# AdaptiveCity/deepdish

Measured on AMD Instinct MI355X. Metric: end-to-end frames/sec (detect+encode+track) at 640x480, higher is better.
Workload: dtype i8 (reference: uint8); encoder f16; 1 GPU; SSD-MobileNet-v1 uint8-quantised (300x300) + MARS-64x32x3 + deep_sort on synthetic 640x480 BGR frames, ~20 synthetic detections/frame (BASELINE.json configs[1]); streams_per_gpu=3072, worker_threads_per_gpu=2, parallelism=independent streams, 3072 per GPU in 2 worker groups, weights=seeded synthetic (seed 1234)

## Files before the change

### deepdish_amd/csrc/mars_pair.hip

```cpp
#include "mars_tail.h"

namespace {

typedef _Float16 h8 __attribute__((ext_vector_type(8)));
typedef float f4 __attribute__((ext_vector_type(4)));
typedef unsigned u4 __attribute__((ext_vector_type(4)));

__device__ __forceinline__ float elu(float v) {
    float e = __builtin_amdgcn_exp2f(v * 1.44269504088896340736f);
    e = __builtin_amdgcn_fmed3f(e, 0.f, 1.f);
    return __builtin_amdgcn_fmed3f(v, e - 1.f, 3.0e38f);
}

__device__ __forceinline__ void lds_fill16(const _Float16 *g, char *lds_wave_base) {
#if defined(__HIP_DEVICE_COMPILE__)
    __builtin_amdgcn_global_load_lds(g, lds_wave_base, 16, 0, 0);
#endif
}

__device__ __forceinline__ int frag_row(int a, int fr) { return (fr >> 2) * 8 + (a & 1) * 4 + (fr & 3); }

constexpr int PZ_B = 3072;
constexpr int PT64_B = 18 * 1024;
constexpr int PT32_B = 33 * 1024;
constexpr int PPLAIN_B = 16 * 1024;
constexpr int PRAW_B = 8 * 1024;
constexpr int pair_off_in(bool) { return PZ_B; }
constexpr int pair_off_h(bool first) { return PZ_B + 2 * (first ? PT32_B : PT64_B); }
constexpr int pair_off_res(bool first) { return pair_off_h(first) + 2 * PT64_B; }
constexpr int pair_off_raw(bool first) { return pair_off_res(first) + (first ? 2 : 3) * PPLAIN_B; }
constexpr int pair_off_const(bool first) { return pair_off_raw(first) + (first ? 2 * PRAW_B : 0); }
constexpr int pair_lds_bytes(bool first) { return pair_off_const(first) + 5 * 64 * 4; }

template <bool FIRST>
__global__ __launch_bounds__(512, 2) void mars_pair64_k(const MarsPairP P) {
    constexpr int OFF_IN = pair_off_in(FIRST), OFF_H = pair_off_h(FIRST), OFF_RES = pair_off_res(FIRST), OFF_RAW = pair_off_raw(FIRST),
                  OFF_C = pair_off_const(FIRST);
    constexpr int TIN_B = FIRST ? PT32_B : PT64_B, NRES = FIRST ? 2 : 3;
    extern __shared__ __attribute__((aligned(16))) char smem[];
    const int tid = threadIdx.x, lane = tid & 63;
    const int wave = __builtin_amdgcn_readfirstlane(tid >> 6);
    const int stage = wave >> 2, half = wave & 1, q = (wave >> 1) & 1;
    const int fr = lane & 15, fq = lane >> 4, j = fr >> 3, x = fr & 7;

    for (int i = tid * 16; i < OFF_C; i += 512 * 16) *reinterpret_cast<u4 *>(smem + i) = u4{0u, 0u, 0u, 0u};
    float *cst = reinterpret_cast<float *>(smem + OFF_C);
    if (tid < 64) {
        cst[tid] = P.bias_a[tid];
        cst[64 + tid] = P.bias_b[tid];
        cst[128 + tid] = P.aff2[tid];
        cst[192 + tid] = P.aff2[P.cout_pad + tid];
        cst[256 + tid] = (FIRST && P.bias_p) ? P.bias_p[tid] : 0.f;
    }
    __syncthreads();

    h8 wf[9][2][2];
    h8 wp[2];
    const bool a32 = FIRST && stage == 0;
    {
        const _Float16 *w = stage == 0 ? P.wa : P.wb;
        const int kpad = stage == 0 ? P.kpad_a : P.kpad_b;
#pragma unroll
        for (int t = 0; t < 9; ++t)
#pragma unroll
            for (int ks = 0; ks < 2; ++ks)
#pragma unroll
                for (int a = 0; a < 2; ++a) {
                    const size_t row = (size_t)(half * 32 + frag_row(a, fr)) * kpad;
                    wf[t][ks][a] = a32 ? *reinterpret_cast<const h8 *>(w + row + t * 32 + fq * 8)
                                       : *reinterpret_cast<const h8 *>(w + row + t * 64 + ks * 32 + fq * 8);
                }
#pragma unroll
        for (int a = 0; a < 2; ++a)
// ... 16 lines not shown
    size_t stp[5];
    int n_dma;
    if constexpr (FIRST) {
        const int par = lane >> 5, pl = (lane >> 3) & 3, col = 2 * (lane & 7) + par;
#pragma unroll
        for (int h = 0; h < 4; ++h) {
            const int r = wave + 8 * h < 31 ? wave + 8 * h : 30;
            src[h] = col < 15 ? P.in + ((size_t)n0 * 31 + r) * 15 * P.cs_in + (size_t)col * P.cs_in + P.coff_in + pl * 8 : P.zero;
            stp[h] = col < 15 ? (size_t)nstep * 31 * 15 * P.cs_in : 0;
        }
        const int jr = lane >> 5, xx = lane & 7;
        src[4] = P.in2 + ((size_t)n0 * 31 + 2 * (2 * wave + jr)) * 15 * P.cs_in2 + (size_t)(2 * xx) * P.cs_in2 + P.coff_in2 + pl * 8;
        stp[4] = (size_t)nstep * 31 * 15 * P.cs_in2;
        n_dma = 5;
    } else {
        const int pl = lane >> 3, xx = lane & 7;
#pragma unroll
        for (int h = 0; h < 2; ++h) {
            src[h] = P.in + (((size_t)n0 * 16 + wave + 8 * h) * 8 + xx) * P.cs_in + P.coff_in + pl * 8;
            stp[h] = (size_t)nstep * 128 * P.cs_in;
            src[2 + h] = P.res + (((size_t)n0 * 16 + wave + 8 * h) * 8 + xx) * P.cs_res + P.coff_res + pl * 8;
            stp[2 + h] = (size_t)nstep * 128 * P.cs_res;
        }
        src[4] = P.zero; stp[4] = 0;
        n_dma = 4;
    }
    (void)n_dma;
    int dq = 0;
    auto issue = [&]() {
        char *T = smem + OFF_IN + (dq & 1) * TIN_B;
        if constexpr (FIRST) {
#pragma unroll
            for (int h = 0; h < 4; ++h) lds_fill16(src[h], T + ((wave + 8 * h < 31 ? wave + 8 * h : 30) + 1) * 1024);
            lds_fill16(src[4], smem + OFF_RAW + (dq & 1) * PRAW_B + wave * 1024);
        } else {
#pragma unroll
            for (int h = 0; h < 2; ++h) lds_fill16(src[h], T + (wave + 8 * h + 1) * 1024);
            const int rs = dq % 3;
#pragma unroll
            for (int h = 0; h < 2; ++h) lds_fill16(src[2 + h], smem + OFF_RES + rs * PPLAIN_B + (wave + 8 * h) * 1024);
        }
        ++dq;
        const bool more = dq < Kc;
#pragma unroll
        for (int h = 0; h < 5; ++h) src[h] += more ? stp[h] : 0;
    };

    const int co = half * 32 + fq * 8;
    const unsigned lo64 = (unsigned)((j * 64 + fq * 8 + x) * 16);
    const unsigned lo32 = (unsigned)((2 * j * 64 + fq * 8 + x) * 16);
    const f4 ba0 = *reinterpret_cast<const f4 *>(cst + (stage ? 64 : 0) + co), ba1 = *reinterpret_cast<const f4 *>(cst + (stage ? 64 : 0) + co + 4);

    issue();
    for (int c = 0; c <= Kc; ++c) {
#if defined(__HIP_DEVICE_COMPILE__)
        if (stage == 0 || c < 2) asm volatile("s_waitcnt vmcnt(0) lgkmcnt(0)" ::: "memory");
        else asm volatile("s_waitcnt vmcnt(8) lgkmcnt(0)" ::: "memory");
        __builtin_amdgcn_s_barrier();
        asm volatile("" ::: "memory");
#endif
        issue();
        const int cc = stage == 0 ? c : c - 1;
        if (cc < 0 || cc >= Kc) continue;
        const size_t n = (size_t)(n0 + cc * nstep);
#pragma unroll 1
        for (int f = 0; f < 4; ++f) {
            const int F = 4 * q + f;
            f4 acc[2] = {f4{0.f, 0.f, 0.f, 0.f}, f4{0.f, 0.f, 0.f, 0.f}};
            h8 X[4];
            if (a32) {
                const unsigned tb = (unsigned)(OFF_IN + (cc & 1) * PT32_B + 4 * F * 1024) + lo32;
                const unsigned bL = x == 0 ? ((tb + 512u - 16u) & 255u) : tb + 512u - 16u, bC = tb, bR = tb + 512u;
                const unsigned pb = (unsigned)(OFF_RAW + (cc & 1) * PRAW_B) + (unsigned)(((2 * F + j) * 32 + fq * 8 + x) * 16);
                f4 accp[2] = {f4{0.f, 0.f, 0.f, 0.f}, f4{0.f, 0.f, 0.f, 0.f}};
#if defined(__HIP_DEVICE_COMPILE__)
#define DD_RD(u_) do { if constexpr ((u_) < 9) { constexpr int dy_ = (u_) / 3, dx_ = (u_) - dy_ * 3;                                               \
                           asm volatile("ds_read_b128 %0, %1 offset:%2" : "=&v"(X[(u_) & 3]) : "v"(dx_ == 0 ? bL : dx_ == 1 ? bC : bR), "n"(dy_ * 1024) : "memory"); } \
                       else asm volatile("ds_read_b128 %0, %1" : "=&v"(X[(u_) & 3]) : "v"(pb) : "memory"); } while (0)
#define DD_UNIT(u_) do { if constexpr ((u_) + 3 < 10) DD_RD(((u_) + 3) % 10);                                                                      \
                         asm volatile("s_waitcnt lgkmcnt(%1)" : "+v"(X[(u_) & 3]) : "n"((u_) + 3 < 10 ? 3 : 9 - (u_)));                           \
                         if constexpr ((u_) < 9) { _Pragma("unroll") for (int a = 0; a < 2; ++a) acc[a] = __builtin_amdgcn_mfma_f32_16x16x32_f16(wf[(u_) % 9][0][a], X[(u_) & 3], acc[a], 0, 0, 0); } \
                         else { _Pragma("unroll") for (int a = 0; a < 2; ++a) accp[a] = __builtin_amdgcn_mfma_f32_16x16x32_f16(wp[a], X[(u_) & 3], accp[a], 0, 0, 0); } } while (0)
                DD_RD(0); DD_RD(1); DD_RD(2);
                DD_UNIT(0); DD_UNIT(1); DD_UNIT(2); DD_UNIT(3); DD_UNIT(4); DD_UNIT(5); DD_UNIT(6); DD_UNIT(7); DD_UNIT(8); DD_UNIT(9);
#undef DD_UNIT
#undef DD_RD
#endif
                const f4 c0 = *reinterpret_cast<const f4 *>(cst + 256 + co), c1 = *reinterpret_cast<const f4 *>(cst + 256 + co + 4);
                h8 sk;
#pragma unroll
                for (int i = 0; i < 4; ++i) { sk[i] = (_Float16)(accp[0][i] + c0[i]); sk[4 + i] = (_Float16)(accp[1][i] + c1[i]); }
                *reinterpret_cast<h8 *>(smem + OFF_RES + (cc & 1) * PPLAIN_B + ((2 * F + j) * 64 + (half * 4 + fq) * 8 + x) * 16) = sk;
            } else {
                const unsigned tb = (unsigned)((stage == 0 ? OFF_IN + (cc & 1) * PT64_B : OFF_H + (cc & 1) * PT64_B) + 2 * F * 1024) + lo64;
                const unsigned bL = x == 0 ? ((tb - 16u) & 255u) : tb - 16u, bC = tb, bR = x == 7 ? ((tb + 16u) & 255u) : tb + 16u;
#if defined(__HIP_DEVICE_COMPILE__)
#define DD_RD(u_) do { constexpr int t_ = (u_) >> 1, ks_ = (u_) & 1, dy_ = t_ / 3, dx_ = t_ - dy_ * 3;                                             \
                       asm volatile("ds_read_b128 %0, %1 offset:%2" : "=&v"(X[(u_) & 3]) : "v"(dx_ == 0 ? bL : dx_ == 1 ? bC : bR), "n"(dy_ * 1024 + ks_ * 512) : "memory"); } while (0)
#define DD_UNIT(u_) do { if constexpr ((u_) + 3 < 18) DD_RD(((u_) + 3) % 18);                                                                      \
                         asm volatile("s_waitcnt lgkmcnt(%1)" : "+v"(X[(u_) & 3]) : "n"((u_) + 3 < 18 ? 3 : 17 - (u_)));                          \
                         _Pragma("unroll") for (int a = 0; a < 2; ++a) acc[a] = __builtin_amdgcn_mfma_f32_16x16x32_f16(wf[(u_) >> 1][(u_) & 1][a], X[(u_) & 3], acc[a], 0, 0, 0); } while (0)
                DD_RD(0); DD_RD(1); DD_RD(2);
                DD_UNIT(0); DD_UNIT(1); DD_UNIT(2); DD_UNIT(3); DD_UNIT(4); DD_UNIT(5); DD_UNIT(6); DD_UNIT(7); DD_UNIT(8);
                DD_UNIT(9); DD_UNIT(10); DD_UNIT(11); DD_UNIT(12); DD_UNIT(13); DD_UNIT(14); DD_UNIT(15); DD_UNIT(16); DD_UNIT(17);
#undef DD_UNIT
#undef DD_RD
#endif
            }
            float v[8];
#pragma unroll
            for (int i = 0; i < 4; ++i) { v[i] = acc[0][i] + ba0[i]; v[4 + i] = acc[1][i] + ba1[i]; }
            if (stage == 0) {
                h8 o;
#pragma unroll
                for (int i = 0; i < 8; ++i) o[i] = (_Float16)elu(v[i]);
                *reinterpret_cast<h8 *>(smem + OFF_H + (cc & 1) * PT64_B + ((2 * F + j + 1) * 64 + (half * 4 + fq) * 8 + x) * 16) = o;
            } else {
                const int rs = FIRST ? (cc & 1) : cc % 3;
                const h8 rv = *reinterpret_cast<const h8 *>(smem + OFF_RES + rs * PPLAIN_B + ((2 * F + j) * 64 + (half * 4 + fq) * 8 + x) * 16);
#pragma unroll
                for (int i = 0; i < 8; ++i) v[i] += (float)rv[i];
                const size_t m = (n * 16 + 2 * F + j) * 8 + x;
                h8 o;
#pragma unroll
                for (int i = 0; i < 8; ++i) o[i] = (_Float16)v[i];
                *reinterpret_cast<h8 *>(P.out + m * P.cs_out + P.coff_out + co) = o;
                const f4 s0 = *reinterpret_cast<const f4 *>(cst + 128 + co), s1 = *reinterpret_cast<const f4 *>(cst + 128 + co + 4);
                const f4 t0 = *reinterpret_cast<const f4 *>(cst + 192 + co), t1 = *reinterpret_cast<const f4 *>(cst + 192 + co + 4);
                h8 o2;
#pragma unroll
                for (int i = 0; i < 4; ++i) { o2[i] = (_Float16)elu(s0[i] * v[i] + t0[i]); o2[4 + i] = (_Float16)elu(s1[i] * v[4 + i] + t1[i]); }
                *reinterpret_cast<h8 *>(P.out2 + m * P.cs_out2 + P.coff_out2 + co) = o2;
            }
        }
    }
#if defined(__HIP_DEVICE_COMPILE__)
    asm volatile("s_waitcnt vmcnt(0)" ::: "memory");
#endif
}

template <bool FIRST>
int launch_pair(hipStream_t s, int device, const MarsPairP &P) {
    constexpr int lds = pair_lds_bytes(FIRST);
    static_assert(lds <= 160 * 1024, "LDS budget");
    static DevOnce once;
    const int rc = once.run(device, [&]() -> int {
        DD_HIP(hipFuncSetAttribute(reinterpret_cast<const void *>(&mars_pair64_k<FIRST>), hipFuncAttributeMaxDynamicSharedMemorySize, lds));
        return DD_OK;
    });
    if (rc != DD_OK) return rc;
    const int n_cu = dd_cu_count(device);
    const int grid = P.n_img < n_cu ? P.n_img : n_cu;
    hipLaunchKernelGGL((mars_pair64_k<FIRST>), dim3(grid), dim3(512), lds, s, P);
    DD_LAUNCH_CHECK();
    return DD_OK;
}

}

int mars_pair64_launch(hipStream_t s, int device, const MarsPairP &P, bool first) {
    DD_REQUIRE(P.n_img > 0 && P.in && P.wa && P.wb && P.bias_a && P.bias_b && P.out && P.out2 && P.aff2 && P.zero && (first ? (P.in2 && P.wp) : P.res != nullptr), DD_E_ARG,
               "mars_pair64: bad argument");
    return first ? launch_pair<true>(s, device, P) : launch_pair<false>(s, device, P);
}
```

### deepdish_amd/csrc/mars_tail.hip

```cpp
#include "mars_tail.h"
#include <vector>

namespace {

typedef _Float16 h8 __attribute__((ext_vector_type(8)));
typedef float f4 __attribute__((ext_vector_type(4)));
typedef unsigned u4 __attribute__((ext_vector_type(4)));

enum { ACT_NONE = 0, ACT_ELU = 2 };

__device__ __forceinline__ float elu(float v) {
    float e = __builtin_amdgcn_exp2f(v * 1.44269504088896340736f);
    e = __builtin_amdgcn_fmed3f(e, 0.f, 1.f);
    return __builtin_amdgcn_fmed3f(v, e - 1.f, 3.0e38f);
}

__device__ __forceinline__ void lds_fill16(const _Float16 *g, char *lds_wave_base) {
#if defined(__HIP_DEVICE_COMPILE__)
    __builtin_amdgcn_global_load_lds(g, lds_wave_base, 16, 0, 0);
#endif
}

__device__ __forceinline__ int frag_row(int a, int fr) { return (fr >> 2) * 8 + (a & 1) * 4 + (fr & 3); }

#ifdef DD_MARS_STAMPS
__device__ unsigned long long dd_mars_stamps[256 * 8 * 8];
#define DD_STAMP(k) do { const unsigned long long t_ = __builtin_amdgcn_s_memtime(); st_acc[k] += t_ - st_last; st_last = t_; } while (0)
#else
#define DD_STAMP(k) do { } while (0)
#endif

constexpr int WS_LEAD = 2, WS_NB = WS_LEAD + 2, WS_NBR = WS_LEAD + 3;
constexpr int ws_tile_bytes(int mode) { return mode == MARS_WS_S2_PROJ ? 17 * 68 * 16 : 10 * 72 * 16; }
constexpr int ws_zero_bytes(int mode) { return mode == MARS_WS_S2_PROJ ? 0 : 7680; }
constexpr int WS_RES_BYTES = 8 * 72 * 16, WS_PRJ_BYTES = 4096;
constexpr int ws_xw_bytes(int mode) { return mode == MARS_WS_S2_PROJ ? 4096 : 2048; }
constexpr int ws_off_tiles(int mode) { return ws_zero_bytes(mode); }
constexpr int ws_off_aux(int mode) { return ws_off_tiles(mode) + WS_NB * ws_tile_bytes(mode); }
constexpr int ws_off_xchg(int mode) {
    return ws_off_aux(mode) + (mode == MARS_WS_S1_RES ? WS_NBR * WS_RES_BYTES : mode == MARS_WS_S2_PROJ ? WS_NB * WS_PRJ_BYTES : 0);
}
constexpr int ws_off_const(int mode) { return ws_off_xchg(mode) + 2 * 8 * ws_xw_bytes(mode); }
constexpr int ws_lds_bytes(int mode) { return ws_off_const(mode) + 3 * 128 * 4; }

template <int MODE, int ACT, bool OUT2>
__global__ __launch_bounds__(512, 2) void mars_ws128_k(const MarsWsP P) {
    constexpr bool S2 = MODE == MARS_WS_S2_PROJ, RES = MODE == MARS_WS_S1_RES;
    constexpr int LEAD = WS_LEAD, NB = WS_NB, NBR = WS_NBR;
    constexpr int TILE_B = ws_tile_bytes(MODE), XW_B = ws_xw_bytes(MODE);
    constexpr int OFF_T = ws_off_tiles(MODE), OFF_A = ws_off_aux(MODE), OFF_X = ws_off_xchg(MODE), OFF_C = ws_off_const(MODE);
    constexpr int KS = S2 ? 1 : 2, CIN = S2 ? 64 : 128;
    [[maybe_unused]] constexpr int N_DMA = S2 ? 3 : RES ? 2 : 1;
    [[maybe_unused]] constexpr int N_ST = S2 ? 2 : (RES && OUT2) ? 2 : 1;
    extern __shared__ __attribute__((aligned(16))) char smem[];
    const int tid = threadIdx.x, lane = tid & 63;
    const int wave = __builtin_amdgcn_readfirstlane(tid >> 6);
    const int cg = wave & 3, kh = wave >> 2;
    const int fr = lane & 15, fq = lane >> 4, yy = fr >> 2, x = fr & 3;

    for (int i = tid * 16; i < OFF_A; i += 512 * 16) *reinterpret_cast<u4 *>(smem + i) = u4{0u, 0u, 0u, 0u};
    float *cst = reinterpret_cast<float *>(smem + OFF_C);
    if (tid < 128) {
        cst[tid] = P.bias[tid];
        if constexpr (S2) cst[128 + tid] = P.bias2 ? P.bias2[tid] : 0.f;
        if constexpr (RES && OUT2) { cst[128 + tid] = P.aff2[tid]; cst[256 + tid] = P.aff2[P.cout_pad + tid]; }
    }
    __syncthreads();

    h8 wf[9][KS][2];
#pragma unroll
    for (int t = 0; t < 9; ++t)
#pragma unroll
        for (int ks = 0; ks < KS; ++ks)
#pragma unroll
            for (int a = 0; a < 2; ++a)
                wf[t][ks][a] = *reinterpret_cast<const h8 *>(P.w + (size_t)(cg * 32 + frag_row(a, fr)) * P.kpad + t * CIN + kh * (CIN / 2) + ks * 32 + fq * 8);
    h8 wp[2];
    if constexpr (S2) {
#pragma unroll
        for (int a = 0; a < 2; ++a) wp[a] = *reinterpret_cast<const h8 *>(P.w2 + (size_t)(cg * 32 + frag_row(a, fr)) * P.kpad2 + kh * 32 + fq * 8);
    }

#if defined(__HIP_DEVICE_COMPILE__)
#pragma unroll
    for (int t = 0; t < 9; ++t)
#pragma unroll
        for (int ks = 0; ks < KS; ++ks)
#pragma unroll
            for (int a = 0; a < 2; ++a) asm volatile("" ::"v"(wf[t][ks][a]));
    if constexpr (S2) asm volatile("" ::"v"(wp[0]), "v"(wp[1]));
#endif

    const int n0 = blockIdx.x, nstep = gridDim.x;
    const int Kc = (P.n_img - n0 + nstep - 1) / nstep;

    int dq = 0, dq_slot = 0, dq_rslot = 0;
    const _Float16 *src_a, *src_b, *src_c;
    size_t step_a, step_b, step_c;
    if constexpr (!S2) {
        src_a = P.in + (size_t)n0 * 32 * P.cs_in + ((wave * 4 + (lane & 3)) * P.cs_in + P.coff_in + (lane >> 2) * 8);
        src_b = RES ? P.res + (size_t)n0 * 32 * P.cs_res + ((wave * 4 + (lane & 3)) * P.cs_res + P.coff_res + (lane >> 2) * 8) : P.zero;
        src_c = P.zero;
        step_a = (size_t)nstep * 32 * P.cs_in; step_b = (size_t)nstep * 32 * P.cs_res; step_c = 0;
    } else {
        const int par = lane >> 5, pl = (lane >> 2) & 7, col = 2 * (lane & 3) + par;
        src_a = P.in + (size_t)n0 * 128 * P.cs_in + ((wave * 8 + col) * P.cs_in + P.coff_in + pl * 8);
        src_b = src_a + (size_t)64 * P.cs_in;
        const int ch = (wave & 3) * 64 + lane;
        src_c = P.in2 + (size_t)n0 * 128 * P.cs_in2 + ((2 * ((ch >> 2) & 7) * 8 + 2 * (ch & 3)) * P.cs_in2 + P.coff_in2 + (ch >> 5) * 8);
        step_a = step_b = (size_t)nstep * 128 * P.cs_in; step_c = (size_t)nstep * 128 * P.cs_in2;
    }
    auto issue = [&]() {
        char *T = smem + OFF_T + dq_slot * TILE_B;
        if constexpr (!S2) {
            lds_fill16(src_a, T + (wave + 1) * 72 * 16);
            if constexpr (RES) lds_fill16(src_b, smem + OFF_A + dq_rslot * WS_RES_BYTES + wave * 72 * 16);
        } else {
            lds_fill16(src_a, T + wave * 68 * 16);
            lds_fill16(src_b, T + (wave + 8) * 68 * 16);
            lds_fill16(src_c, smem + OFF_A + dq_slot * WS_PRJ_BYTES + (wave & 3) * 1024);
        }
        ++dq;
        const bool more = dq < Kc;
        src_a += more ? step_a : 0;
        if constexpr (RES || S2) src_b += more ? step_b : 0;
        if constexpr (S2) src_c += more ? step_c : 0;
        dq_slot = dq_slot + 1 == NB ? 0 : dq_slot + 1;
        dq_rslot = dq_rslot + 1 == NBR ? 0 : dq_rslot + 1;
    };

    const unsigned lo = S2 ? (unsigned)((2 * yy * 68 + (kh * 4 + fq) * 4 + x) * 16) : (unsigned)((yy * 72 + (kh * 8 + fq) * 4 + x) * 16);
    const unsigned lo_prj = (unsigned)(((kh * 4 + fq) * 32 + yy * 4 + x) * 16);
    const unsigned lo_res = (unsigned)(((4 * kh + yy) * 72 + (cg * 4 + fq) * 4 + x) * 16);
    const int co = cg * 32 + fq * 8;
    const f4 b0 = *reinterpret_cast<const f4 *>(cst + co), b1 = *reinterpret_cast<const f4 *>(cst + co + 4);

    f4 keep[S2 ? 4 : 2];
    int slot = 0, rslot_prev = 0, rslot = 0;

    auto epilogue = [&](int cprev) {
        const char *Xp = smem + OFF_X + ((cprev & 1) * 8 + (wave ^ 4)) * XW_B + lane * 16;
        const size_t n = (size_t)(n0 + cprev * nstep);
        const size_t m = (n * 8 + 4 * kh + yy) * 4 + x;
        float v[8];
        {
            const f4 o0 = *reinterpret_cast<const f4 *>(Xp), o1 = *reinterpret_cast<const f4 *>(Xp + 1024);
#pragma unroll
            for (int i = 0; i < 4; ++i) { v[i] = keep[0][i] + o0[i] + b0[i]; v[4 + i] = keep[1][i] + o1[i] + b1[i]; }
        }
        if constexpr (ACT == ACT_ELU) {
#pragma unroll
            for (int i = 0; i < 8; ++i) v[i] = elu(v[i]);
        }
        if constexpr (RES) {
            const h8 rv = *reinterpret_cast<const h8 *>(smem + OFF_A + rslot_prev * WS_RES_BYTES + lo_res);
#pragma unroll
            for (int i = 0; i < 8; ++i) v[i] += (float)rv[i];
        }
        h8 o;
#pragma unroll
        for (int i = 0; i < 8; ++i) o[i] = (_Float16)v[i];
        *reinterpret_cast<h8 *>(P.out + m * P.cs_out + P.coff_out + co) = o;
        if constexpr (RES && OUT2) {
            const f4 s0 = *reinterpret_cast<const f4 *>(cst + 128 + co), s1 = *reinterpret_cast<const f4 *>(cst + 128 + co + 4);
            const f4 t0 = *reinterpret_cast<const f4 *>(cst + 256 + co), t1 = *reinterpret_cast<const f4 *>(cst + 256 + co + 4);
            h8 o2;
#pragma unroll
            for (int i = 0; i < 4; ++i) { o2[i] = (_Float16)elu(s0[i] * v[i] + t0[i]); o2[4 + i] = (_Float16)elu(s1[i] * v[4 + i] + t1[i]); }
            *reinterpret_cast<h8 *>(P.out2 + m * P.cs_out2 + P.coff_out2 + co) = o2;
        }
        if constexpr (S2) {
            const f4 o0 = *reinterpret_cast<const f4 *>(Xp + 2048), o1 = *reinterpret_cast<const f4 *>(Xp + 3072);
            const f4 c0 = *reinterpret_cast<const f4 *>(cst + 128 + co), c1 = *reinterpret_cast<const f4 *>(cst + 128 + co + 4);
            h8 o2;
#pragma unroll
            for (int i = 0; i < 4; ++i) { o2[i] = (_Float16)(keep[2][i] + o0[i] + c0[i]); o2[4 + i] = (_Float16)(keep[3][i] + o1[i] + c1[i]); }
            *reinterpret_cast<h8 *>(P.out2 + m * P.cs_out2 + P.coff_out2 + co) = o2;
        }
    };

#ifdef DD_MARS_STAMPS
    unsigned long long st_acc[8] = {0, 0, 0, 0, 0, 0, 0, 0}, st_last = __builtin_amdgcn_s_memtime();
    const unsigned long long st_begin = st_last;
#endif
    static_assert(LEAD == 2, "the counted waits below are written for two crops of look-ahead");
    for (int ci = 0; ci < LEAD; ++ci) issue();
    DD_STAMP(0);
    for (int c = 0; c <= Kc; ++c) {
#if defined(__HIP_DEVICE_COMPILE__)
        if (kh == 0 || c == 0) {
            if (c <= 1) asm volatile("s_waitcnt vmcnt(%0) lgkmcnt(0)" ::"i"(N_DMA) : "memory");
            else if (c == 2) asm volatile("s_waitcnt vmcnt(%0) lgkmcnt(0)" ::"i"(N_DMA + N_ST) : "memory");
            else asm volatile("s_waitcnt vmcnt(%0) lgkmcnt(0)" ::"i"(N_DMA + 2 * N_ST) : "memory");
        } else asm volatile("s_waitcnt lgkmcnt(0)" ::: "memory");
        DD_STAMP(2);
        __builtin_amdgcn_s_barrier();
        asm volatile("" ::: "memory");
#endif
        DD_STAMP(3);
        auto compute = [&](f4 (&kp)[S2 ? 4 : 2]) {
            const unsigned tb = (unsigned)(OFF_T + slot * TILE_B) + lo;
            f4 acc[2][2] = {{f4{0.f, 0.f, 0.f, 0.f}, f4{0.f, 0.f, 0.f, 0.f}}, {f4{0.f, 0.f, 0.f, 0.f}, f4{0.f, 0.f, 0.f, 0.f}}};
            if constexpr (!S2) {
                const unsigned bs[3] = {x == 0 ? ((tb - 16u) & 255u) : tb - 16u, tb, x == 3 ? ((tb + 16u) & 255u) : tb + 16u};
                h8 X[4][2];
#if defined(__HIP_DEVICE_COMPILE__)
#define DD_RD(u_) do { constexpr int t_ = (u_) >> 1, p_ = (u_) & 1, dy_ = t_ / 3, dx_ = t_ - dy_ * 3;                                      \
                       asm volatile("ds_read_b128 %0, %2 offset:%3\n\tds_read_b128 %1, %2 offset:%4"                                       \
                                    : "=&v"(X[(u_) & 3][0]), "=&v"(X[(u_) & 3][1]) : "v"(bs[dx_]), "n"(((4 * p_ + dy_) * 72) * 16), "n"(((4 * p_ + dy_) * 72 + 16) * 16) : "memory"); } while (0)
#define DD_UNIT(u_) do { if constexpr ((u_) + 3 < 18) DD_RD(((u_) + 3) % 18);                                                            \
                         asm volatile("s_waitcnt lgkmcnt(%2)" : "+v"(X[(u_) & 3][0]), "+v"(X[(u_) & 3][1]) : "n"((u_) + 3 < 18 ? 6 : 2 * (17 - (u_))));          \
                         _Pragma("unroll") for (int ks = 0; ks < 2; ++ks) _Pragma("unroll") for (int a = 0; a < 2; ++a)                  \
                             acc[(u_) & 1][a] = __builtin_amdgcn_mfma_f32_16x16x32_f16(wf[(u_) >> 1][ks][a], X[(u_) & 3][ks], acc[(u_) & 1][a], 0, 0, 0); } while (0)
                DD_RD(0); DD_RD(1); DD_RD(2);
                DD_UNIT(0); DD_UNIT(1); DD_UNIT(2); DD_UNIT(3); DD_UNIT(4); DD_UNIT(5); DD_UNIT(6); DD_UNIT(7); DD_UNIT(8);
                DD_UNIT(9); DD_UNIT(10); DD_UNIT(11); DD_UNIT(12); DD_UNIT(13); DD_UNIT(14); DD_UNIT(15); DD_UNIT(16); DD_UNIT(17);
#undef DD_UNIT
#undef DD_RD
#endif
            } else {
                f4 accp[2][2] = {{f4{0.f, 0.f, 0.f, 0.f}, f4{0.f, 0.f, 0.f, 0.f}}, {f4{0.f, 0.f, 0.f, 0.f}, f4{0.f, 0.f, 0.f, 0.f}}};
                h8 X[4];
                const unsigned pb = (unsigned)(OFF_A + slot * WS_PRJ_BYTES) + lo_prj;
                const h8 hz = {(_Float16)0.f, (_Float16)0.f, (_Float16)0.f, (_Float16)0.f, (_Float16)0.f, (_Float16)0.f, (_Float16)0.f, (_Float16)0.f};
#if defined(__HIP_DEVICE_COMPILE__)
#define DD_RD(u_) do { if constexpr ((u_) < 18) { constexpr int t_ = (u_) >> 1, p_ = (u_) & 1, dy_ = t_ / 3, dx_ = t_ - dy_ * 3;                    \
                           asm volatile("ds_read_b128 %0, %1 offset:%2" : "=&v"(X[(u_) & 3]) : "v"(tb), "n"(((8 * p_ + dy_) * 68 + (dx_ == 1 ? 32 : 0) + (dx_ == 2 ? 1 : 0)) * 16) : "memory"); } \
                       else asm volatile("ds_read_b128 %0, %1 offset:%2" : "=&v"(X[(u_) & 3]) : "v"(pb), "n"(((u_) - 18) * 256) : "memory"); } while (0)
#define DD_UNIT(u_) do { if constexpr ((u_) + 3 < 20) DD_RD(((u_) + 3) % 20);                                                            \
                         asm volatile("s_waitcnt lgkmcnt(%1)" : "+v"(X[(u_) & 3]) : "n"((u_) + 3 < 20 ? 3 : 19 - (u_)));               \
                         if constexpr ((u_) < 18) { const h8 xv_ = (((u_) >> 1) % 3 == 2 && x == 3) ? hz : X[(u_) & 3];                    \
                             _Pragma("unroll") for (int a = 0; a < 2; ++a) acc[(u_) & 1][a] = __builtin_amdgcn_mfma_f32_16x16x32_f16(wf[(u_) >> 1][0][a], xv_, acc[(u_) & 1][a], 0, 0, 0); } \
                         else { _Pragma("unroll") for (int a = 0; a < 2; ++a) accp[(u_) - 18][a] = __builtin_amdgcn_mfma_f32_16x16x32_f16(wp[a], X[(u_) & 3], accp[(u_) - 18][a], 0, 0, 0); } } while (0)
                DD_RD(0); DD_RD(1); DD_RD(2);
                DD_UNIT(0); DD_UNIT(1); DD_UNIT(2); DD_UNIT(3); DD_UNIT(4); DD_UNIT(5); DD_UNIT(6); DD_UNIT(7); DD_UNIT(8); DD_UNIT(9);
                DD_UNIT(10); DD_UNIT(11); DD_UNIT(12); DD_UNIT(13); DD_UNIT(14); DD_UNIT(15); DD_UNIT(16); DD_UNIT(17); DD_UNIT(18); DD_UNIT(19);
#undef DD_UNIT
#undef DD_RD
#endif
                char *Xm = smem + OFF_X + ((c & 1) * 8 + wave) * XW_B + lane * 16;
                *reinterpret_cast<f4 *>(Xm + 2048) = kh ? accp[0][0] : accp[1][0];
                *reinterpret_cast<f4 *>(Xm + 3072) = kh ? accp[0][1] : accp[1][1];
                kp[2] = kh ? accp[1][0] : accp[0][0];
                kp[3] = kh ? accp[1][1] : accp[0][1];
            }
            char *Xm = smem + OFF_X + ((c & 1) * 8 + wave) * XW_B + lane * 16;
            *reinterpret_cast<f4 *>(Xm) = kh ? acc[0][0] : acc[1][0];
            *reinterpret_cast<f4 *>(Xm + 1024) = kh ? acc[0][1] : acc[1][1];
            kp[0] = kh ? acc[1][0] : acc[0][0];
            kp[1] = kh ? acc[1][1] : acc[0][1];
        };
        if (kh == 0) {
            f4 kn[S2 ? 4 : 2];
            if (c < Kc) compute(kn);
            DD_STAMP(5);
#if defined(__HIP_DEVICE_COMPILE__)
            asm volatile("s_waitcnt lgkmcnt(0)" ::: "memory");
            __builtin_amdgcn_s_barrier();
            asm volatile("" ::: "memory");
#endif
            DD_STAMP(3);
            issue();
            DD_STAMP(1);
            if (c > 0) epilogue(c - 1);
            DD_STAMP(4);
#pragma unroll
            for (int i = 0; i < (S2 ? 4 : 2); ++i) keep[i] = kn[i];
        } else {
            issue();
            DD_STAMP(1);
            if (c > 0) epilogue(c - 1);
            DD_STAMP(4);
#if defined(__HIP_DEVICE_COMPILE__)
            if (c == 0) asm volatile("s_waitcnt vmcnt(%0) lgkmcnt(0)" ::"i"(N_DMA) : "memory");
            else if (c == 1) asm volatile("s_waitcnt vmcnt(%0) lgkmcnt(0)" ::"i"(N_DMA + N_ST) : "memory");
            else asm volatile("s_waitcnt vmcnt(%0) lgkmcnt(0)" ::"i"(N_DMA + 2 * N_ST) : "memory");
            __builtin_amdgcn_s_barrier();
            asm volatile("" ::: "memory");
#endif
            DD_STAMP(3);
            if (c < Kc) compute(keep);
            DD_STAMP(5);
        }
        slot = slot + 1 == NB ? 0 : slot + 1;
        rslot_prev = rslot;
        rslot = rslot + 1 == NBR ? 0 : rslot + 1;
    }
#if defined(__HIP_DEVICE_COMPILE__)
    asm volatile("s_waitcnt vmcnt(0)" ::: "memory");
#endif
#ifdef DD_MARS_STAMPS
    if (lane == 0) {
        unsigned long long *d = dd_mars_stamps + ((size_t)blockIdx.x * 8 + wave) * 8;
        for (int k = 0; k < 6; ++k) d[k] = st_acc[k];
        d[6] = __builtin_amdgcn_s_memtime() - st_begin;
        d[7] = (unsigned long long)Kc;
    }
#endif
}

template <int MODE, int ACT, bool OUT2>
int launch_one(hipStream_t s, int device, const MarsWsP &P) {
    constexpr int lds = ws_lds_bytes(MODE);
    static_assert(lds <= 160 * 1024, "LDS budget");
    static DevOnce once;
    const int rc = once.run(device, [&]() -> int {
        DD_HIP(hipFuncSetAttribute(reinterpret_cast<const void *>(&mars_ws128_k<MODE, ACT, OUT2>), hipFuncAttributeMaxDynamicSharedMemorySize, lds));
        return DD_OK;
    });
    if (rc != DD_OK) return rc;
    const int n_cu = dd_cu_count(device);
    const int grid = P.n_img < n_cu ? P.n_img : n_cu;
    hipLaunchKernelGGL((mars_ws128_k<MODE, ACT, OUT2>), dim3(grid), dim3(512), lds, s, P);
    DD_LAUNCH_CHECK();
#ifdef DD_MARS_STAMPS
    {
        static std::vector<unsigned long long> h(256 * 8 * 8);
        DD_HIP(hipStreamSynchronize(s));
        DD_HIP(hipMemcpyFromSymbol(h.data(), HIP_SYMBOL(dd_mars_stamps), h.size() * 8));
        for (int half = 0; half < 2; ++half) {
            double a[7] = {0, 0, 0, 0, 0, 0, 0};
            int nw = 0;
            for (int b = 0; b < grid; ++b)
                for (int w = half * 4; w < half * 4 + 4; ++w, ++nw) {
                    const unsigned long long *d = h.data() + ((size_t)b * 8 + w) * 8;
                    for (int k = 0; k < 7; ++k) a[k] += (double)d[k] / (double)(k == 0 || k == 6 ? 1 : d[7] + 1);
                }
            fprintf(stderr, "mars_ws128_k<%d,%d,%d> K half %d: prologue DMAs %.0f | per step: issue %.0f, wait %.0f, barrier %.0f, epilogue %.0f, compute %.0f | loop total %.0f cycles, %d steps\n",
                    MODE, ACT, (int)OUT2, half, a[0] / nw, a[1] / nw, a[2] / nw, a[3] / nw, a[4] / nw, a[5] / nw, a[6] / nw, (int)h[7] + 1);
        }
    }
#endif
    return DD_OK;
}

}

int mars_ws128_launch(hipStream_t s, int device, const MarsWsP &P, int mode, int act, bool out2) {
    DD_REQUIRE(P.n_img > 0 && P.in && P.w && P.bias && P.out && P.zero, DD_E_ARG, "mars_ws128: bad argument");
    DD_REQUIRE((long long)P.n_img * 128 * (P.cs_in > P.cs_out ? P.cs_in : P.cs_out) < (1ll << 40), DD_E_CAPACITY, "mars_ws128: batch of %d", P.n_img);
    if (mode == MARS_WS_S2_PROJ) {
        DD_REQUIRE(P.in2 && P.w2 && P.out2 && act == ACT_ELU, DD_E_ARG, "mars_ws128: stride-2 form needs the projection operands and ELU");
        return launch_one<MARS_WS_S2_PROJ, ACT_ELU, false>(s, device, P);
    }
    if (mode == MARS_WS_S1) {
        DD_REQUIRE(!P.res && !P.out2, DD_E_ARG, "mars_ws128: plain form with a residual or a second output");
        return act == ACT_ELU ? launch_one<MARS_WS_S1, ACT_ELU, false>(s, device, P) : launch_one<MARS_WS_S1, ACT_NONE, false>(s, device, P);
    }
    DD_REQUIRE(mode == MARS_WS_S1_RES && P.res && act == ACT_NONE && (!out2 || (P.out2 && P.aff2)), DD_E_ARG, "mars_ws128: residual form");
    return out2 ? launch_one<MARS_WS_S1_RES, ACT_NONE, true>(s, device, P) : launch_one<MARS_WS_S1_RES, ACT_NONE, false>(s, device, P);
}
```

Measured before the change: 145,300 frames/s.

## Process two crops per pipeline step in stride-1 MARS 128-channel conv kernel

Adds a template parameter NC so each loop iteration of the stride-1 warp-specialised 128-channel conv handles two crops. Barriers and waits are amortised over twice the MFMA work, and the DMA look-ahead and residual lag are restructured to match. NC=2 is the default, selectable through DD_MARS_STEP_CROPS. This raises LDS use and register pressure (two keep sets, reloaded bias), which could lower occupancy. Timing stamps are also added to the pair kernel under a debug macro.

```diff
diff --git a/deepdish_amd/csrc/mars_pair.hip b/deepdish_amd/csrc/mars_pair.hip
--- a/deepdish_amd/csrc/mars_pair.hip
+++ b/deepdish_amd/csrc/mars_pair.hip
@@ -1,4 +1,5 @@
 #include "mars_tail.h"
+#include <vector>
 
 namespace {
 
@@ -19,6 +20,10 @@
 }
 
 __device__ __forceinline__ int frag_row(int a, int fr) { return (fr >> 2) * 8 + (a & 1) * 4 + (fr & 3); }
+
+#ifdef DD_MARS_STAMPS
+__device__ unsigned long long dd_pair_stamps[256 * 8 * 4];
+#endif
 
 constexpr int PZ_B = 3072;
 constexpr int PT64_B = 18 * 1024;
@@ -141,12 +146,22 @@
     const f4 ba0 = *reinterpret_cast<const f4 *>(cst + (stage ? 64 : 0) + co), ba1 = *reinterpret_cast<const f4 *>(cst + (stage ? 64 : 0) + co + 4);
 
     issue();
+#ifdef DD_MARS_STAMPS
+    unsigned long long st_wait = 0, st_work = 0, st_last = __builtin_amdgcn_s_memtime();
+    const unsigned long long st_begin = st_last;
+#endif
     for (int c = 0; c <= Kc; ++c) {
+#ifdef DD_MARS_STAMPS
+        { const unsigned long long t_ = __builtin_amdgcn_s_memtime(); st_work += t_ - st_last; st_last = t_; }
+#endif
 #if defined(__HIP_DEVICE_COMPILE__)
         if (stage == 0 || c < 2) asm volatile("s_waitcnt vmcnt(0) lgkmcnt(0)" ::: "memory");
         else asm volatile("s_waitcnt vmcnt(8) lgkmcnt(0)" ::: "memory");
         __builtin_amdgcn_s_barrier();
         asm volatile("" ::: "memory");
+#endif
+#ifdef DD_MARS_STAMPS
+        { const unsigned long long t_ = __builtin_amdgcn_s_memtime(); st_wait += t_ - st_last; st_last = t_; }
 #endif
         issue();
         const int cc = stage == 0 ? c : c - 1;
@@ -226,6 +241,12 @@
 #if defined(__HIP_DEVICE_COMPILE__)
     asm volatile("s_waitcnt vmcnt(0)" ::: "memory");
 #endif
+#ifdef DD_MARS_STAMPS
+    if (lane == 0 && blockIdx.x < 256) {
+        unsigned long long *d = dd_pair_stamps + ((size_t)blockIdx.x * 8 + wave) * 4;
+        d[0] = st_wait; d[1] = st_work; d[2] = __builtin_amdgcn_s_memtime() - st_begin; d[3] = (unsigned long long)Kc;
+    }
+#endif
 }
 
 template <bool FIRST>
@@ -242,6 +263,25 @@
     const int grid = P.n_img < n_cu ? P.n_img : n_cu;
     hipLaunchKernelGGL((mars_pair64_k<FIRST>), dim3(grid), dim3(512), lds, s, P);
     DD_LAUNCH_CHECK();
+#ifdef DD_MARS_STAMPS
+    {
+        static std::vector<unsigned long long> h(256 * 8 * 4);
+        DD_HIP(hipStreamSynchronize(s));
+        DD_HIP(hipMemcpyFromSymbol(h.data(), HIP_SYMBOL(dd_pair_stamps), h.size() * 8));
+        const int nb = grid < 256 ? grid : 256;
+        for (int stage = 0; stage < 2; ++stage) {
+            double a[3] = {0, 0, 0};
+            int nw = 0;
+            for (int b = 0; b < nb; ++b)
+                for (int w = stage * 4; w < stage * 4 + 4; ++w, ++nw) {
+                    const unsigned long long *d = h.data() + ((size_t)b * 8 + w) * 4;
+                    a[0] += (double)d[0] / (double)(d[3] + 1); a[1] += (double)d[1] / (double)(d[3] + 1); a[2] += (double)d[2];
+                }
+            fprintf(stderr, "mars_pair64_k<%d> stage %c: per step: wait + barrier %.0f, issue + compute + epilogue %.0f | loop total %.0f cycles, %d steps\n",
+                    (int)FIRST, stage ? 'B' : 'A', a[0] / nw, a[1] / nw, a[2] / nw, (int)h[3] + 1);
+        }
+    }
+#endif
     return DD_OK;
 }
 
diff --git a/deepdish_amd/csrc/mars_tail.hip b/deepdish_amd/csrc/mars_tail.hip
--- a/deepdish_amd/csrc/mars_tail.hip
+++ b/deepdish_amd/csrc/mars_tail.hip
@@ -30,25 +30,29 @@
 #define DD_STAMP(k) do { } while (0)
 #endif
 
-constexpr int WS_LEAD = 2, WS_NB = WS_LEAD + 2, WS_NBR = WS_LEAD + 3;
+constexpr int ws_lead(int nc) { return nc == 1 ? 2 : 1; }
+constexpr int ws_rlag(int nc) { return nc == 1 ? 0 : 1; }
+constexpr int ws_nb(int nc) { return nc == 1 ? 4 : 2; }
+constexpr int ws_nbr(int nc) { return nc == 1 ? 5 : 2; }
 constexpr int ws_tile_bytes(int mode) { return mode == MARS_WS_S2_PROJ ? 17 * 68 * 16 : 10 * 72 * 16; }
 constexpr int ws_zero_bytes(int mode) { return mode == MARS_WS_S2_PROJ ? 0 : 7680; }
 constexpr int WS_RES_BYTES = 8 * 72 * 16, WS_PRJ_BYTES = 4096;
 constexpr int ws_xw_bytes(int mode) { return mode == MARS_WS_S2_PROJ ? 4096 : 2048; }
 constexpr int ws_off_tiles(int mode) { return ws_zero_bytes(mode); }
-constexpr int ws_off_aux(int mode) { return ws_off_tiles(mode) + WS_NB * ws_tile_bytes(mode); }
-constexpr int ws_off_xchg(int mode) {
-    return ws_off_aux(mode) + (mode == MARS_WS_S1_RES ? WS_NBR * WS_RES_BYTES : mode == MARS_WS_S2_PROJ ? WS_NB * WS_PRJ_BYTES : 0);
-}
-constexpr int ws_off_const(int mode) { return ws_off_xchg(mode) + 2 * 8 * ws_xw_bytes(mode); }
-constexpr int ws_lds_bytes(int mode) { return ws_off_const(mode) + 3 * 128 * 4; }
-
-template <int MODE, int ACT, bool OUT2>
+constexpr int ws_off_aux(int mode, int nc) { return ws_off_tiles(mode) + nc * ws_nb(nc) * ws_tile_bytes(mode); }
+constexpr int ws_off_xchg(int mode, int nc) {
+    return ws_off_aux(mode, nc) + (mode == MARS_WS_S1_RES ? nc * ws_nbr(nc) * WS_RES_BYTES : mode == MARS_WS_S2_PROJ ? nc * ws_nb(nc) * WS_PRJ_BYTES : 0);
+}
+constexpr int ws_off_const(int mode, int nc) { return ws_off_xchg(mode, nc) + 2 * nc * 8 * ws_xw_bytes(mode); }
+constexpr int ws_lds_bytes(int mode, int nc) { return ws_off_const(mode, nc) + 3 * 128 * 4; }
+
+template <int MODE, int ACT, bool OUT2, int NC>
 __global__ __launch_bounds__(512, 2) void mars_ws128_k(const MarsWsP P) {
     constexpr bool S2 = MODE == MARS_WS_S2_PROJ, RES = MODE == MARS_WS_S1_RES;
-    constexpr int LEAD = WS_LEAD, NB = WS_NB, NBR = WS_NBR;
+    constexpr int LEAD = ws_lead(NC), RLAG = ws_rlag(NC), NB = NC * ws_nb(NC), NBR = NC * ws_nbr(NC);
     constexpr int TILE_B = ws_tile_bytes(MODE), XW_B = ws_xw_bytes(MODE);
-    constexpr int OFF_T = ws_off_tiles(MODE), OFF_A = ws_off_aux(MODE), OFF_X = ws_off_xchg(MODE), OFF_C = ws_off_const(MODE);
+    constexpr int OFF_T = ws_off_tiles(MODE), OFF_A = ws_off_aux(MODE, NC), OFF_X = ws_off_xchg(MODE, NC), OFF_C = ws_off_const(MODE, NC);
+    constexpr int KP = S2 ? 4 : 2;
     constexpr int KS = S2 ? 1 : 2, CIN = S2 ? 64 : 128;
     [[maybe_unused]] constexpr int N_DMA = S2 ? 3 : RES ? 2 : 1;
     [[maybe_unused]] constexpr int N_ST = S2 ? 2 : (RES && OUT2) ? 2 : 1;
@@ -94,7 +98,8 @@
     const int n0 = blockIdx.x, nstep = gridDim.x;
     const int Kc = (P.n_img - n0 + nstep - 1) / nstep;
 
-    int dq = 0, dq_slot = 0, dq_rslot = 0;
+    const int Ks = (Kc + NC - 1) / NC;
+    int dq = 0, dq_slot = 0, dr = 0, dr_slot = 0;
     const _Float16 *src_a, *src_b, *src_c;
     size_t step_a, step_b, step_c;
     if constexpr (!S2) {
@@ -110,11 +115,10 @@
         src_c = P.in2 + (size_t)n0 * 128 * P.cs_in2 + ((2 * ((ch >> 2) & 7) * 8 + 2 * (ch & 3)) * P.cs_in2 + P.coff_in2 + (ch >> 5) * 8);
         step_a = step_b = (size_t)nstep * 128 * P.cs_in; step_c = (size_t)nstep * 128 * P.cs_in2;
     }
-    auto issue = [&]() {
+    auto issue_tile = [&]() {
         char *T = smem + OFF_T + dq_slot * TILE_B;
         if constexpr (!S2) {
             lds_fill16(src_a, T + (wave + 1) * 72 * 16);
-            if constexpr (RES) lds_fill16(src_b, smem + OFF_A + dq_rslot * WS_RES_BYTES + wave * 72 * 16);
         } else {
             lds_fill16(src_a, T + wave * 68 * 16);
             lds_fill16(src_b, T + (wave + 8) * 68 * 16);
@@ -123,27 +127,43 @@
         ++dq;
         const bool more = dq < Kc;
         src_a += more ? step_a : 0;
-        if constexpr (RES || S2) src_b += more ? step_b : 0;
-        if constexpr (S2) src_c += more ? step_c : 0;
+        if constexpr (S2) { src_b += more ? step_b : 0; src_c += more ? step_c : 0; }
         dq_slot = dq_slot + 1 == NB ? 0 : dq_slot + 1;
-        dq_rslot = dq_rslot + 1 == NBR ? 0 : dq_rslot + 1;
+    };
+    auto issue_res = [&]() {
+        if constexpr (RES) {
+            lds_fill16(src_b, smem + OFF_A + dr_slot * WS_RES_BYTES + wave * 72 * 16);
+            ++dr;
+            src_b += dr < Kc ? step_b : 0;
+            dr_slot = dr_slot + 1 == NBR ? 0 : dr_slot + 1;
+        }
+    };
+    auto issue = [&]() {
+#pragma unroll
+        for (int j = 0; j < NC; ++j) { issue_tile(); issue_res(); }
     };
 
     const unsigned lo = S2 ? (unsigned)((2 * yy * 68 + (kh * 4 + fq) * 4 + x) * 16) : (unsigned)((yy * 72 + (kh * 8 + fq) * 4 + x) * 16);
     const unsigned lo_prj = (unsigned)(((kh * 4 + fq) * 32 + yy * 4 + x) * 16);
     const unsigned lo_res = (unsigned)(((4 * kh + yy) * 72 + (cg * 4 + fq) * 4 + x) * 16);
     const int co = cg * 32 + fq * 8;
-    const f4 b0 = *reinterpret_cast<const f4 *>(cst + co), b1 = *reinterpret_cast<const f4 *>(cst + co + 4);
-
-    f4 keep[S2 ? 4 : 2];
+    const int co_lane = co;
+    const f4 b0_reg = *reinterpret_cast<const f4 *>(cst + co), b1_reg = *reinterpret_cast<const f4 *>(cst + co + 4);
+
+    f4 keep[NC][KP];
     int slot = 0, rslot_prev = 0, rslot = 0;
 
-    auto epilogue = [&](int cprev) {
-        const char *Xp = smem + OFF_X + ((cprev & 1) * 8 + (wave ^ 4)) * XW_B + lane * 16;
+    auto epilogue = [&](int cprev, int xs, int rs, const f4 (&keep)[KP]) {
+        const char *Xp = smem + OFF_X + (xs * 8 + (wave ^ 4)) * XW_B + lane * 16;
         const size_t n = (size_t)(n0 + cprev * nstep);
         const size_t m = (n * 8 + 4 * kh + yy) * 4 + x;
+        int co = co_lane;
+#if defined(__HIP_DEVICE_COMPILE__)
+        if constexpr (NC == 2) asm volatile("" : "+v"(co));
+#endif
         float v[8];
         {
+            const f4 b0 = NC == 1 ? b0_reg : *reinterpret_cast<const f4 *>(cst + co), b1 = NC == 1 ? b1_reg : *reinterpret_cast<const f4 *>(cst + co + 4);
             const f4 o0 = *reinterpret_cast<const f4 *>(Xp), o1 = *reinterpret_cast<const f4 *>(Xp + 1024);
 #pragma unroll
             for (int i = 0; i < 4; ++i) { v[i] = keep[0][i] + o0[i] + b0[i]; v[4 + i] = keep[1][i] + o1[i] + b1[i]; }
@@ -153,7 +173,7 @@
             for (int i = 0; i < 8; ++i) v[i] = elu(v[i]);
         }
         if constexpr (RES) {
-            const h8 rv = *reinterpret_cast<const h8 *>(smem + OFF_A + rslot_prev * WS_RES_BYTES + lo_res);
+            const h8 rv = *reinterpret_cast<const h8 *>(smem + OFF_A + rs * WS_RES_BYTES + lo_res);
 #pragma unroll
             for (int i = 0; i < 8; ++i) v[i] += (float)rv[i];
         }
@@ -183,38 +203,65 @@
     unsigned long long st_acc[8] = {0, 0, 0, 0, 0, 0, 0, 0}, st_last = __builtin_amdgcn_s_memtime();
     const unsigned long long st_begin = st_last;
 #endif
-    static_assert(LEAD == 2, "the counted waits below are written for two crops of look-ahead");
-    for (int ci = 0; ci < LEAD; ++ci) issue();
+    static_assert((NC == 1 && LEAD == 2 && RLAG == 0) || (NC == 2 && LEAD == 1 && RLAG == 1 && !S2), "the counted waits below are written for these two schedules");
+#pragma unroll
+    for (int ci = 0; ci < LEAD * NC; ++ci) {
+        issue_tile();
+        if (ci < (LEAD - RLAG) * NC) issue_res();
+    }
     DD_STAMP(0);
-    for (int c = 0; c <= Kc; ++c) {
-#if defined(__HIP_DEVICE_COMPILE__)
-        if (kh == 0 || c == 0) {
-            if (c <= 1) asm volatile("s_waitcnt vmcnt(%0) lgkmcnt(0)" ::"i"(N_DMA) : "memory");
-            else if (c == 2) asm volatile("s_waitcnt vmcnt(%0) lgkmcnt(0)" ::"i"(N_DMA + N_ST) : "memory");
-            else asm volatile("s_waitcnt vmcnt(%0) lgkmcnt(0)" ::"i"(N_DMA + 2 * N_ST) : "memory");
-        } else asm volatile("s_waitcnt lgkmcnt(0)" ::: "memory");
+    for (int c = 0; c <= Ks; ++c) {
+#if defined(__HIP_DEVICE_COMPILE__)
+        if constexpr (NC == 1) {
+            if (kh == 0 || c == 0) {
+                if (c <= 1) asm volatile("s_waitcnt vmcnt(%0) lgkmcnt(0)" ::"i"(N_DMA) : "memory");
+                else if (c == 2) asm volatile("s_waitcnt vmcnt(%0) lgkmcnt(0)" ::"i"(N_DMA + N_ST) : "memory");
+                else asm volatile("s_waitcnt vmcnt(%0) lgkmcnt(0)" ::"i"(N_DMA + 2 * N_ST) : "memory");
+            } else asm volatile("s_waitcnt lgkmcnt(0)" ::: "memory");
+        } else {
+            if (c <= 1) asm volatile("s_waitcnt vmcnt(0) lgkmcnt(0)" ::: "memory");
+            else asm volatile("s_waitcnt vmcnt(%0) lgkmcnt(0)" ::"i"(NC * N_ST) : "memory");
+        }
         DD_STAMP(2);
         __builtin_amdgcn_s_barrier();
         asm volatile("" ::: "memory");
 #endif
         DD_STAMP(3);
-        auto compute = [&](f4 (&kp)[S2 ? 4 : 2]) {
+        auto compute = [&](f4 (&kp)[NC][KP]) {
             const unsigned tb = (unsigned)(OFF_T + slot * TILE_B) + lo;
             f4 acc[2][2] = {{f4{0.f, 0.f, 0.f, 0.f}, f4{0.f, 0.f, 0.f, 0.f}}, {f4{0.f, 0.f, 0.f, 0.f}, f4{0.f, 0.f, 0.f, 0.f}}};
+            auto hand_over = [&](int j_) {
+                char *Xm = smem + OFF_X + (((c & 1) * NC + j_) * 8 + wave) * XW_B + lane * 16;
+                *reinterpret_cast<f4 *>(Xm) = kh ? acc[0][0] : acc[1][0];
+                *reinterpret_cast<f4 *>(Xm + 1024) = kh ? acc[0][1] : acc[1][1];
+                kp[j_][0] = kh ? acc[1][0] : acc[0][0];
+                kp[j_][1] = kh ? acc[1][1] : acc[0][1];
+            };
             if constexpr (!S2) {
-                const unsigned bs[3] = {x == 0 ? ((tb - 16u) & 255u) : tb - 16u, tb, x == 3 ? ((tb + 16u) & 255u) : tb + 16u};
+                const unsigned tb1 = tb + (unsigned)((NC - 1) * TILE_B);
+                const unsigned bs[2][3] = {{x == 0 ? ((tb - 16u) & 255u) : tb - 16u, tb, x == 3 ? ((tb + 16u) & 255u) : tb + 16u},
+                                           {x == 0 ? ((tb1 - 16u) & 255u) : tb1 - 16u, tb1, x == 3 ? ((tb1 + 16u) & 255u) : tb1 + 16u}};
                 h8 X[4][2];
 #if defined(__HIP_DEVICE_COMPILE__)
-#define DD_RD(u_) do { constexpr int t_ = (u_) >> 1, p_ = (u_) & 1, dy_ = t_ / 3, dx_ = t_ - dy_ * 3;                                      \
+#define DD_RD(u_) do { constexpr int j_ = (u_) / 18, t_ = ((u_) % 18) >> 1, p_ = (u_) & 1, dy_ = t_ / 3, dx_ = t_ - dy_ * 3;                \
                        asm volatile("ds_read_b128 %0, %2 offset:%3\n\tds_read_b128 %1, %2 offset:%4"                                       \
-                                    : "=&v"(X[(u_) & 3][0]), "=&v"(X[(u_) & 3][1]) : "v"(bs[dx_]), "n"(((4 * p_ + dy_) * 72) * 16), "n"(((4 * p_ + dy_) * 72 + 16) * 16) : "memory"); } while (0)
-#define DD_UNIT(u_) do { if constexpr ((u_) + 3 < 18) DD_RD(((u_) + 3) % 18);                                                            \
-                         asm volatile("s_waitcnt lgkmcnt(%2)" : "+v"(X[(u_) & 3][0]), "+v"(X[(u_) & 3][1]) : "n"((u_) + 3 < 18 ? 6 : 2 * (17 - (u_))));          \
+                                    : "=&v"(X[(u_) & 3][0]), "=&v"(X[(u_) & 3][1]) : "v"(bs[j_][dx_]), "n"(((4 * p_ + dy_) * 72) * 16), "n"(((4 * p_ + dy_) * 72 + 16) * 16) : "memory"); } while (0)
+#define DD_UNIT(u_) do { if constexpr ((u_) + 3 < 18 * NC) DD_RD(((u_) + 3) % (18 * NC));                                                \
+                         asm volatile("s_waitcnt lgkmcnt(%2)" : "+v"(X[(u_) & 3][0]), "+v"(X[(u_) & 3][1]) : "n"((u_) + 3 < 18 * NC ? 6 : 2 * (18 * NC - 1 - (u_))));          \
                          _Pragma("unroll") for (int ks = 0; ks < 2; ++ks) _Pragma("unroll") for (int a = 0; a < 2; ++a)                  \
-                             acc[(u_) & 1][a] = __builtin_amdgcn_mfma_f32_16x16x32_f16(wf[(u_) >> 1][ks][a], X[(u_) & 3][ks], acc[(u_) & 1][a], 0, 0, 0); } while (0)
+                             acc[(u_) & 1][a] = __builtin_amdgcn_mfma_f32_16x16x32_f16(wf[((u_) % 18) >> 1][ks][a], X[(u_) & 3][ks], acc[(u_) & 1][a], 0, 0, 0); } while (0)
                 DD_RD(0); DD_RD(1); DD_RD(2);
                 DD_UNIT(0); DD_UNIT(1); DD_UNIT(2); DD_UNIT(3); DD_UNIT(4); DD_UNIT(5); DD_UNIT(6); DD_UNIT(7); DD_UNIT(8);
                 DD_UNIT(9); DD_UNIT(10); DD_UNIT(11); DD_UNIT(12); DD_UNIT(13); DD_UNIT(14); DD_UNIT(15); DD_UNIT(16); DD_UNIT(17);
+                if constexpr (NC == 2) {
+                    hand_over(0);
+#pragma unroll
+                    for (int p = 0; p < 2; ++p)
+#pragma unroll
+                        for (int a = 0; a < 2; ++a) acc[p][a] = f4{0.f, 0.f, 0.f, 0.f};
+                    DD_UNIT(18); DD_UNIT(19); DD_UNIT(20); DD_UNIT(21); DD_UNIT(22); DD_UNIT(23); DD_UNIT(24); DD_UNIT(25); DD_UNIT(26);
+                    DD_UNIT(27); DD_UNIT(28); DD_UNIT(29); DD_UNIT(30); DD_UNIT(31); DD_UNIT(32); DD_UNIT(33); DD_UNIT(34); DD_UNIT(35);
+                }
 #undef DD_UNIT
 #undef DD_RD
 #endif
@@ -241,18 +288,22 @@
                 char *Xm = smem + OFF_X + ((c & 1) * 8 + wave) * XW_B + lane * 16;
                 *reinterpret_cast<f4 *>(Xm + 2048) = kh ? accp[0][0] : accp[1][0];
                 *reinterpret_cast<f4 *>(Xm + 3072) = kh ? accp[0][1] : accp[1][1];
-                kp[2] = kh ? accp[1][0] : accp[0][0];
-                kp[3] = kh ? accp[1][1] : accp[0][1];
+                kp[0][KP - 2] = kh ? accp[1][0] : accp[0][0];
+                kp[0][KP - 1] = kh ? accp[1][1] : accp[0][1];
             }
-            char *Xm = smem + OFF_X + ((c & 1) * 8 + wave) * XW_B + lane * 16;
-            *reinterpret_cast<f4 *>(Xm) = kh ? acc[0][0] : acc[1][0];
-            *reinterpret_cast<f4 *>(Xm + 1024) = kh ? acc[0][1] : acc[1][1];
-            kp[0] = kh ? acc[1][0] : acc[0][0];
-            kp[1] = kh ? acc[1][1] : acc[0][1];
+            hand_over(NC - 1);
+        };
+        auto finish = [&]() {
+            if (c > 0) {
+#pragma unroll
+                for (int j = 0; j < NC; ++j)
+                    if (j == 0 || (c - 1) * NC + j < Kc) epilogue((c - 1) * NC + j, ((c - 1) & 1) * NC + j, rslot_prev + j, keep[j]);
+            }
         };
         if (kh == 0) {
-            f4 kn[S2 ? 4 : 2];
-            if (c < Kc) compute(kn);
+            if constexpr (NC > 1) { issue(); DD_STAMP(1); }
+            f4 kn[NC][KP];
+            if (c < Ks) compute(kn);
             DD_STAMP(5);
 #if defined(__HIP_DEVICE_COMPILE__)
             asm volatile("s_waitcnt lgkmcnt(0)" ::: "memory");
@@ -260,31 +311,34 @@
             asm volatile("" ::: "memory");
 #endif
             DD_STAMP(3);
-            issue();
-            DD_STAMP(1);
-            if (c > 0) epilogue(c - 1);
+            if constexpr (NC == 1) { issue(); DD_STAMP(1); }
+            finish();
             DD_STAMP(4);
 #pragma unroll
-            for (int i = 0; i < (S2 ? 4 : 2); ++i) keep[i] = kn[i];
+            for (int j = 0; j < NC; ++j)
+#pragma unroll
+                for (int i = 0; i < KP; ++i) keep[j][i] = kn[j][i];
         } else {
             issue();
             DD_STAMP(1);
-            if (c > 0) epilogue(c - 1);
+            finish();
             DD_STAMP(4);
 #if defined(__HIP_DEVICE_COMPILE__)
-            if (c == 0) asm volatile("s_waitcnt vmcnt(%0) lgkmcnt(0)" ::"i"(N_DMA) : "memory");
-            else if (c == 1) asm volatile("s_waitcnt vmcnt(%0) lgkmcnt(0)" ::"i"(N_DMA + N_ST) : "memory");
-            else asm volatile("s_waitcnt vmcnt(%0) lgkmcnt(0)" ::"i"(N_DMA + 2 * N_ST) : "memory");
+            if constexpr (NC == 1) {
+                if (c == 0) asm volatile("s_waitcnt vmcnt(%0) lgkmcnt(0)" ::"i"(N_DMA) : "memory");
+                else if (c == 1) asm volatile("s_waitcnt vmcnt(%0) lgkmcnt(0)" ::"i"(N_DMA + N_ST) : "memory");
+                else asm volatile("s_waitcnt vmcnt(%0) lgkmcnt(0)" ::"i"(N_DMA + 2 * N_ST) : "memory");
+            } else asm volatile("s_waitcnt lgkmcnt(0)" ::: "memory");
             __builtin_amdgcn_s_barrier();
             asm volatile("" ::: "memory");
 #endif
             DD_STAMP(3);
-            if (c < Kc) compute(keep);
+            if (c < Ks) compute(keep);
             DD_STAMP(5);
         }
-        slot = slot + 1 == NB ? 0 : slot + 1;
+        slot = slot + NC == NB ? 0 : slot + NC;
         rslot_prev = rslot;
-        rslot = rslot + 1 == NBR ? 0 : rslot + 1;
+        rslot = rslot + NC == NBR ? 0 : rslot + NC;
     }
 #if defined(__HIP_DEVICE_COMPILE__)
     asm volatile("s_waitcnt vmcnt(0)" ::: "memory");
@@ -294,24 +348,24 @@
         unsigned long long *d = dd_mars_stamps + ((size_t)blockIdx.x * 8 + wave) * 8;
         for (int k = 0; k < 6; ++k) d[k] = st_acc[k];
         d[6] = __builtin_amdgcn_s_memtime() - st_begin;
-        d[7] = (unsigned long long)Kc;
-    }
-#endif
-}
-
-template <int MODE, int ACT, bool OUT2>
+        d[7] = (unsigned long long)Ks;
+    }
+#endif
+}
+
+template <int MODE, int ACT, bool OUT2, int NC>
 int launch_one(hipStream_t s, int device, const MarsWsP &P) {
-    constexpr int lds = ws_lds_bytes(MODE);
+    constexpr int lds = ws_lds_bytes(MODE, NC);
     static_assert(lds <= 160 * 1024, "LDS budget");
     static DevOnce once;
     const int rc = once.run(device, [&]() -> int {
-        DD_HIP(hipFuncSetAttribute(reinterpret_cast<const void *>(&mars_ws128_k<MODE, ACT, OUT2>), hipFuncAttributeMaxDynamicSharedMemorySize, lds));
+        DD_HIP(hipFuncSetAttribute(reinterpret_cast<const void *>(&mars_ws128_k<MODE, ACT, OUT2, NC>), hipFuncAttributeMaxDynamicSharedMemorySize, lds));
         return DD_OK;
     });
     if (rc != DD_OK) return rc;
     const int n_cu = dd_cu_count(device);
     const int grid = P.n_img < n_cu ? P.n_img : n_cu;
-    hipLaunchKernelGGL((mars_ws128_k<MODE, ACT, OUT2>), dim3(grid), dim3(512), lds, s, P);
+    hipLaunchKernelGGL((mars_ws128_k<MODE, ACT, OUT2, NC>), dim3(grid), dim3(512), lds, s, P);
     DD_LAUNCH_CHECK();
 #ifdef DD_MARS_STAMPS
     {
@@ -326,8 +380,8 @@
                     const unsigned long long *d = h.data() + ((size_t)b * 8 + w) * 8;
                     for (int k = 0; k < 7; ++k) a[k] += (double)d[k] / (double)(k == 0 || k == 6 ? 1 : d[7] + 1);
                 }
-            fprintf(stderr, "mars_ws128_k<%d,%d,%d> K half %d: prologue DMAs %.0f | per step: issue %.0f, wait %.0f, barrier %.0f, epilogue %.0f, compute %.0f | loop total %.0f cycles, %d steps\n",
-                    MODE, ACT, (int)OUT2, half, a[0] / nw, a[1] / nw, a[2] / nw, a[3] / nw, a[4] / nw, a[5] / nw, a[6] / nw, (int)h[7] + 1);
+            fprintf(stderr, "mars_ws128_k<%d,%d,%d,%d> K half %d: prologue DMAs %.0f | per step: issue %.0f, wait %.0f, barrier %.0f, epilogue %.0f, compute %.0f | loop total %.0f cycles, %d steps\n",
+                    MODE, ACT, (int)OUT2, NC, half, a[0] / nw, a[1] / nw, a[2] / nw, a[3] / nw, a[4] / nw, a[5] / nw, a[6] / nw, (int)h[7] + 1);
         }
     }
 #endif
@@ -341,12 +395,15 @@
     DD_REQUIRE((long long)P.n_img * 128 * (P.cs_in > P.cs_out ? P.cs_in : P.cs_out) < (1ll << 40), DD_E_CAPACITY, "mars_ws128: batch of %d", P.n_img);
     if (mode == MARS_WS_S2_PROJ) {
         DD_REQUIRE(P.in2 && P.w2 && P.out2 && act == ACT_ELU, DD_E_ARG, "mars_ws128: stride-2 form needs the projection operands and ELU");
-        return launch_one<MARS_WS_S2_PROJ, ACT_ELU, false>(s, device, P);
-    }
+        return launch_one<MARS_WS_S2_PROJ, ACT_ELU, false, 1>(s, device, P);
+    }
+    static const bool one = dd_env_int("DD_MARS_STEP_CROPS", 2) == 1;
     if (mode == MARS_WS_S1) {
         DD_REQUIRE(!P.res && !P.out2, DD_E_ARG, "mars_ws128: plain form with a residual or a second output");
-        return act == ACT_ELU ? launch_one<MARS_WS_S1, ACT_ELU, false>(s, device, P) : launch_one<MARS_WS_S1, ACT_NONE, false>(s, device, P);
+        if (one) return act == ACT_ELU ? launch_one<MARS_WS_S1, ACT_ELU, false, 1>(s, device, P) : launch_one<MARS_WS_S1, ACT_NONE, false, 1>(s, device, P);
+        return act == ACT_ELU ? launch_one<MARS_WS_S1, ACT_ELU, false, 2>(s, device, P) : launch_one<MARS_WS_S1, ACT_NONE, false, 2>(s, device, P);
     }
     DD_REQUIRE(mode == MARS_WS_S1_RES && P.res && act == ACT_NONE && (!out2 || (P.out2 && P.aff2)), DD_E_ARG, "mars_ws128: residual form");
-    return out2 ? launch_one<MARS_WS_S1_RES, ACT_NONE, true>(s, device, P) : launch_one<MARS_WS_S1_RES, ACT_NONE, false>(s, device, P);
-}
+    if (one) return out2 ? launch_one<MARS_WS_S1_RES, ACT_NONE, true, 1>(s, device, P) : launch_one<MARS_WS_S1_RES, ACT_NONE, false, 1>(s, device, P);
+    return out2 ? launch_one<MARS_WS_S1_RES, ACT_NONE, true, 2>(s, device, P) : launch_one<MARS_WS_S1_RES, ACT_NONE, false, 2>(s, device, P);
+}
```

Measured after the change: 146,700 frames/s, median of 4. No clear change (+1.0%).
